# Yukun-Huang/DreamWaltz-G

Measured on AMD Instinct MI355X. Metric: SDS steps/sec @512^2, 100k Gaussians, SD1.5+ControlNet; raster Mpix/s vs HBM roofline, higher is better.
Workload: dtype f32x

## Files before the change

### dreamwaltz-g_amd/csrc/gemm.hip

```cpp
#include "dwg_common.h"
#include "dwg_prof_internal.h"
#include "../../include/dwg_gemm.h"
#include <cstdlib>
#include <type_traits>

#if defined(DWG_GEMM_X_TU)
#include "dwg_xfmt.h"
typedef _Float16 HT;
#define DWG_DTYPE_HALF DWG_DTYPE_F32X
#define DWG_MFMA16(a, b, c) __builtin_amdgcn_mfma_f32_32x32x16_f16(a, b, c, 0, 0, 0)
#define DWG_HALF_NAME "f32x"
#elif defined(DWG_GEMM_F16_TU)
typedef _Float16 HT;
#define DWG_DTYPE_HALF DWG_DTYPE_F16
#define DWG_MFMA16(a, b, c) __builtin_amdgcn_mfma_f32_32x32x16_f16(a, b, c, 0, 0, 0)
#define DWG_HALF_NAME "f16"
#else
typedef __bf16 HT;
#define DWG_DTYPE_HALF DWG_DTYPE_BF16
#define DWG_MFMA16(a, b, c) __builtin_amdgcn_mfma_f32_32x32x16_bf16(a, b, c, 0, 0, 0)
#define DWG_HALF_NAME "bf16"
#endif

namespace {

typedef __attribute__((ext_vector_type(8))) HT bf16x8;
typedef __attribute__((ext_vector_type(16))) float f32x16;

struct ConvP {
    int enabled, Cin, Hin, Win, Hout, Wout, KH, KW, stride, pad_t, pad_l, dil;
    int up;
    int cin1;
    const void* A2;
};

struct GemmP {
    const void* A; const void* B; void* C; const void* bias; const void* residual;
    int M, N, K;
    long long sam, sak, sbn, sbk, ldc, ldr;
    int nb2;
    long long bA1, bA2, bB1, bB2, bC1, bC2, bR1, bR2;
    int act; float alpha;
    int out_bf16, res_bf16, bias_per_row, splitk, accumulate;
    float* ws;
    int bias_row_div;
    long long bias_ld;
    ConvP conv;
};

__device__ __forceinline__ float bf2f(HT x) { return (float)x; }
__device__ __forceinline__ HT f2bf(float x) { return (HT)x; }

struct bf16x4_t { HT v[4]; };
#ifdef DWG_GEMM_X_TU
__device__ __forceinline__ float ld_half1(const void* base, long long i) { return dwg_x_get1(base, i); }
__device__ __forceinline__ void st_half1(void* base, long long i, float v) { dwg_x_put1(base, i, v); }
__device__ __forceinline__ void ld_half4(const void* base, long long i, float (&v)[4]) { dwg_x_get4(base, i, v); }
__device__ __forceinline__ void st_half4(void* base, long long i, const float (&v)[4]) { dwg_x_put4(base, i, v); }
#else
__device__ __forceinline__ float ld_half1(const void* base, long long i) { return bf2f(reinterpret_cast<const HT*>(base)[i]); }
__device__ __forceinline__ void st_half1(void* base, long long i, float v) { reinterpret_cast<HT*>(base)[i] = f2bf(v); }
__device__ __forceinline__ void ld_half4(const void* base, long long i, float (&v)[4]) {
    const bf16x4_t r = *reinterpret_cast<const bf16x4_t*>(reinterpret_cast<const HT*>(base) + i);
#pragma unroll
    for (int e = 0; e < 4; e++) v[e] = bf2f(r.v[e]);
}
__device__ __forceinline__ void st_half4(void* base, long long i, const float (&v)[4]) {
    bf16x4_t o;
#pragma unroll
    for (int e = 0; e < 4; e++) o.v[e] = f2bf(v[e]);
    *reinterpret_cast<bf16x4_t*>(reinterpret_cast<HT*>(base) + i) = o;
}
#endif

template <bool LIGHT = false>
__device__ __forceinline__ float apply_act(float v, int act) {
    if constexpr (LIGHT) return act == 3 ? v / (1.f + __expf(-v)) : v;
    switch (act) {
        case 1: return v > 0.f ? v : 0.f;
        case 2: return v > 0.f ? v : 0.01f * v;
        case 3: return v / (1.f + __expf(-v));
        case 4: return 0.5f * v * (1.f + erff(v * 0.70710678118654752f));
        case 5: return 1.f / (1.f + __expf(-v));
        default: return v;
    }
// ... 1058 lines not shown
                if (TAP0 || tap <= NBS - 2) {
                    constexpr int N = (NBS - 2) * NJW + PPW;
                    __builtin_amdgcn_s_waitcnt((N & 15) | ((N >> 4) << 14) | (7 << 4) | (0 << 8));
                } else {
                    constexpr int N = (NBS - 2) * NJW;
                    __builtin_amdgcn_s_waitcnt((N & 15) | ((N >> 4) << 14) | (7 << 4) | (0 << 8));
                }
                __builtin_amdgcn_s_barrier();
                const int ntap = tap == 8 ? 0 : tap + 1;
                const int nty = ntap >= 6 ? 2 : (ntap >= 3 ? 1 : 0);
                load_frags(tap == 8 ? pan : pa, nty * WP + (ntap - 3 * nty), sB + bnext * BBYTES, 0, F[0]);
            }
            __builtin_amdgcn_sched_barrier(0);
            if (ks == 0) {
                const int ft = tap + NBS - 1, fcc = cc + (ft >= 9 ? 1 : 0), ftap = ft >= 9 ? ft - 9 : ft;
                issue_w(fcc, ftap, fcc < ncc, sB + bfill * BBYTES);
                if (TAP0) issue_patch(cc + 1, cc + 1 < ncc, const_cast<unsigned char*>(pan));
            }
            mma(F[ks & 1]);
            if (ks == 0) {
                constexpr int NL = NJW + (TAP0 ? PPW : 0);
#pragma unroll
                for (int m = 0; m < MPS; m++) {
                    __builtin_amdgcn_sched_group_barrier(0x008, 1, 0);
                    __builtin_amdgcn_sched_group_barrier(0x006, (NL * 8 + MPS - 1) / MPS, 0);
                    __builtin_amdgcn_sched_group_barrier(0x020, (NL + MPS - 1) / MPS, 0);
                }
            }
            __builtin_amdgcn_sched_barrier(0);
        }
        __builtin_amdgcn_s_waitcnt(0xC07F);
        bst = bnext;
    };
    for (int cc = cc0; cc < ncc; cc++) {
        const unsigned char* pa = sP + (cc & 1) * PBYTES;
        const unsigned char* pan = sP + ((cc + 1) & 1) * PBYTES;
        step(BoolC<true>{}, 0, cc, pa, pan);
#pragma unroll 1
        for (int tap = 1; tap < 9; tap++) step(BoolC<false>{}, tap, cc, pa, pan);
    }
    wait_vmcnt<0>();
    __builtin_amdgcn_s_barrier();
#ifdef DWG_GEMM_X_TU
#pragma unroll
    for (int i = 0; i < TM; i++)
#pragma unroll
        for (int j = 0; j < TN; j++)
#pragma unroll
            for (int r = 0; r < 16; r++) acc[i][j][r] = fmaf(acx[i][j][r], DWG_X_LO_INV, acc[i][j][r]);
#endif
    constexpr int NPASS = EpiLds<BN, BM>::passes((size_t)2 * PBYTES + NBS * BBYTES);
    static_assert((size_t)2 * PBYTES + NBS * BBYTES >= EpiLds<BN, BM>::bytes(NPASS), "epilogue staging fits in the patch / weight buffers");
    tile_epilogue_lds<BN, NPASS, TM, TN, !SPLIT, BM, NT>(p, acc, reinterpret_cast<float*>(smem_raw), n0, wm, wn, lane, tid, ks_id, 0, 0, [&](int rr) {
        const int y = y0 + rr / PW, x = x0 + rr % PW;
        return (y < cv.Hout && x < cv.Wout) ? (img * cv.Hout + y) * cv.Wout + x : -1;
    });
}

template <int BN, int NW, int NBS>
static void launch_conv3x3_patch2(const GemmP& p, hipStream_t stream, const char* name) {
    typedef Patch2Geom<BN, NW> G;
    const size_t lds = (size_t)2 * G::PBYTES + (size_t)NBS * G::BBYTES;
    const ConvP& cv = p.conv;
    const int nimg = p.M / (cv.Hout * cv.Wout);
    const int gm = nimg * ((cv.Hout + G::PH - 1) / G::PH) * ((cv.Wout + G::PW - 1) / G::PW);
    dim3 grid(gm * ((p.N + BN - 1) / BN) * (p.splitk > 1 ? p.splitk : 1));
    static bool attr_set = false;
    if (!attr_set) {
        hipFuncSetAttribute(reinterpret_cast<const void*>(&k_conv3x3_patch2<BN, false, NW, NBS>), hipFuncAttributeMaxDynamicSharedMemorySize, (int)lds);
        hipFuncSetAttribute(reinterpret_cast<const void*>(&k_conv3x3_patch2<BN, true, NW, NBS>), hipFuncAttributeMaxDynamicSharedMemorySize, (int)lds);
        attr_set = true;
    }
    static_assert((NW == 8 && BN == 128 && NBS == 4) || (NW == 4 && BN == 64 && NBS == 4) || (NW == 4 && BN == 128 && NBS == 2), "symbol table below");
    const char* sym = NW == 8 ? (p.splitk > 1 && p.ws ? "k_conv3x3_patch2<128, true, 8, 4>" : "k_conv3x3_patch2<128, false, 8, 4>")
                              : (BN == 64 ? (p.splitk > 1 && p.ws ? "k_conv3x3_patch2<64, true, 4, 4>" : "k_conv3x3_patch2<64, false, 4, 4>")
                                          : (p.splitk > 1 && p.ws ? "k_conv3x3_patch2<128, true, 4, 2>" : "k_conv3x3_patch2<128, false, 4, 2>"));
    if (p.splitk > 1 && p.ws)
        DWG_LAUNCH_W(name, sym, gemm_flops(p, 1), (k_conv3x3_patch2<BN, true, NW, NBS>), grid, dim3(NW * 64), lds, stream, p);
    else
        DWG_LAUNCH_W(name, sym, gemm_flops(p, 1), (k_conv3x3_patch2<BN, false, NW, NBS>), grid, dim3(NW * 64), lds, stream, p);
    launch_splitk_epilogue(p, stream);
}

template <typename T, int BN, int AMODE, int BMODE>
static void launch(const GemmP& p, int batch, hipStream_t stream, const char* name) {
    constexpr int LDT = TT<T>::BK + TT<T>::PAD;
    size_t lds = (size_t)2 * (128 + BN) * LDT * sizeof(T);
    dim3 grid((p.M + 127) / 128, ((p.N + BN - 1) / BN) * (p.splitk > 1 ? p.splitk : 1), batch);
    static bool attr_set = false;
    if (!attr_set) {
        hipFuncSetAttribute(reinterpret_cast<const void*>(&k_gemm<T, BN, AMODE, BMODE>), hipFuncAttributeMaxDynamicSharedMemorySize,
                            (int)lds);
        attr_set = true;
    }
    DWG_LAUNCH_W(name, (sizeof(T) == 2 ? "k_gemm<" DWG_HALF_NAME ">" : "k_gemm<f32>"), gemm_flops(p, batch), (k_gemm<T, BN, AMODE, BMODE>), grid,
                 dim3(256), lds, stream, p);
    launch_splitk_epilogue(p, stream);
}

template <typename T, int BN, int AMODE>
static void dispatch_b(const GemmP& p, int bmode, int batch, hipStream_t s, const char* name) {
    if (bmode == MODE_KVEC) launch<T, BN, AMODE, MODE_KVEC>(p, batch, s, name);
    else if (bmode == MODE_RVEC) launch<T, BN, AMODE, MODE_RVEC>(p, batch, s, name);
    else launch<T, BN, AMODE, MODE_SCALAR>(p, batch, s, name);
}
template <typename T, int BN>
static void dispatch_a(const GemmP& p, int amode, int bmode, int batch, hipStream_t s, const char* name) {
    if (amode == MODE_KVEC) dispatch_b<T, BN, MODE_KVEC>(p, bmode, batch, s, name);
    else if (amode == MODE_RVEC) dispatch_b<T, BN, MODE_RVEC>(p, bmode, batch, s, name);
    else if (amode == MODE_CONV) dispatch_b<T, BN, MODE_CONV>(p, bmode, batch, s, name);
    else dispatch_b<T, BN, MODE_SCALAR>(p, bmode, batch, s, name);
}

static int batch_of(const dwg_gemm_desc* d) { return d->batch1 * d->batch2; }

static int tile_bn(const dwg_gemm_desc* d) {
    if (d->N <= 64) return 64;
    const long long blocks128 = (long long)((d->M + 127) / 128) * ((d->N + 127) / 128) * batch_of(d);
    return blocks128 < 256 ? 64 : 128;
}

constexpr int kCUs = 256, kMinWgs = 200;
static bool fills_cus(long long wgs) {
    const long long rounds = (wgs + kCUs - 1) / kCUs;
    return wgs >= kMinWgs && wgs * 100 >= rounds * kCUs * 80;
}

constexpr int kSplitkTarget = 256;
constexpr int kSplitkNoSplit = 384;
constexpr int kSplitkMinSteps = 12;
static int auto_splitk(int M, int N, int K, int bn, int bk) {
    long long blocks = (long long)((M + 127) / 128) * ((N + bn - 1) / bn);
    if (blocks >= kSplitkNoSplit || K < 2 * kSplitkMinSteps * bk) return 1;
    if (2.0 * M * N * K < 4.0e8) return 1;
    long long sk = kSplitkTarget / blocks;
    long long kmax = K / (kSplitkMinSteps * bk);
    if (sk > kmax) sk = kmax;
    if (sk > 16) sk = 16;
    return sk >= 2 ? (int)sk : 1;
}

constexpr int kBigMinK = 1280, kBigMaxTiles = 2048;
constexpr int kBigMinSteps = 8, kBigSkMax = 24;
static int big_tile(int M, int N, int K, int* splitk_out) {
    *splitk_out = 1;
    if (K < kBigMinK) return 0;
    int bm = 0;
    if (M >= 192) { if (N >= 128 && (N % 128 == 0 || N >= 640)) bm = 256; }
    else if (N >= 256) bm = 128;
    if (!bm) return 0;
    const int bn = bm == 256 ? 128 : 256;
    const long long tiles = (long long)((M + bm - 1) / bm) * ((N + bn - 1) / bn);
    if (tiles > kBigMaxTiles) return 0;
    long long sk = 1;
    if (tiles < kCUs) {
        sk = kCUs / tiles;
        const long long kmax = K / (kBigMinSteps * 64);
        if (sk > kmax) sk = kmax;
        if (sk > kBigSkMax) sk = kBigSkMax;
        if (sk < 1) sk = 1;
    }
    if (!fills_cus(tiles * sk)) return 0;
    *splitk_out = (int)sk;
    return bm;
}

template <typename T>
static int pick_mode(const void* base, long long srow, long long sk, int nrows, int K, const long long* boffs, int nboffs) {
    constexpr int VEC = TT<T>::VEC;
    bool aligned = ((uintptr_t)base % 16) == 0;
    for (int i = 0; i < nboffs; i++) aligned = aligned && (boffs[i] % VEC == 0);
    if (sk == 1 && aligned && K % VEC == 0 && srow % VEC == 0) return MODE_KVEC;
    if (srow == 1 && aligned && nrows % VEC == 0 && sk % VEC == 0) return MODE_RVEC;
    return MODE_SCALAR;
}

static int splitk_of(const dwg_gemm_desc* d) {
    if (d->splitk > 1) return d->splitk;
    if (d->splitk != 0 || d->act == DWG_ACT_GEGLU_PAIR) return 1;
    return auto_splitk(d->M, d->N, d->K, tile_bn(d), d->dtype == DWG_DTYPE_HALF ? TT<HT>::BK : TT<float>::BK);
}
static bool slabs_possible(const dwg_gemm_desc* d) { return batch_of(d) == 1 && (long long)d->M * d->N < (1LL << 33); }
static long long fit_workspace(const dwg_gemm_desc* d, long long sk) {
    while (sk > 1 && (size_t)sk * d->M * d->N * sizeof(float) > d->workspace_bytes) sk--;
    return sk;
}

enum Family { FAM_GENERIC, FAM_GLDS, FAM_GLDS8, FAM_PATCH2 };
struct Plan {
    Family fam;
    int bm, bn, nw;
    int amode, bmode;
    int akind;
    int splitk;
    bool slabs;
};

constexpr int kPatchMinM = 8192;
constexpr int kPatch8MinSteps = 100;

static int make_plan(const dwg_gemm_desc* d, const GemmP& p, Plan& pl) {
    const bool half = d->dtype == DWG_DTYPE_HALF;
#if defined(DWG_GEMM_F16_TU) || defined(DWG_GEMM_X_TU)
    if (!half) return DWG_E_ARG;
#endif
    pl = Plan{FAM_GENERIC, 128, tile_bn(d), 4, MODE_KVEC, MODE_KVEC, 0, d->splitk > 1 ? d->splitk : 1, false};
    if (d->workspace && slabs_possible(d)) {
        pl.splitk = (int)fit_workspace(d, splitk_of(d));
        pl.slabs = pl.splitk > 1;
    }
    const long long ao[2] = {p.bA1, p.bA2}, bo[2] = {p.bB1, p.bB2};
    if (p.conv.enabled) {
        const int vec = half ? TT<HT>::VEC : TT<float>::VEC;
        if (d->conv_cin % vec != 0 || ((uintptr_t)d->A % 16) != 0) return DWG_E_ARG;
        if (d->A2 && (d->conv_cin1 % vec != 0 || d->conv_cin1 <= 0 || d->conv_cin1 >= d->conv_cin || ((uintptr_t)d->A2 % 16) != 0))
            return DWG_E_ARG;
        if (d->K != d->conv_kh * d->conv_kw * d->conv_cin) return DWG_E_ARG;
        pl.amode = MODE_CONV;
    } else {
        pl.amode = half ? pick_mode<HT>(p.A, p.sam, p.sak, p.M, p.K, ao, 2) : pick_mode<float>(p.A, p.sam, p.sak, p.M, p.K, ao, 2);
    }
    pl.bmode = half ? pick_mode<HT>(p.B, p.sbn, p.sbk, p.N, p.K, bo, 2) : pick_mode<float>(p.B, p.sbn, p.sbk, p.N, p.K, bo, 2);
    if (!half) return DWG_OK;
    if (pl.bmode != MODE_KVEC || (pl.amode != MODE_KVEC && pl.amode != MODE_CONV)) {
#ifdef DWG_GEMM_X_TU
        return DWG_E_ARG;
#else
        return DWG_OK;
#endif
    }
    const ConvP& cv = p.conv;
    const char* minm = getenv("DWG_CONV_PATCH_MINM");
    const int patch_min_m = minm ? atoi(minm) : kPatchMinM;
    const bool patch_geom = pl.amode == MODE_CONV && batch_of(d) == 1 && d->conv_kh == 3 && d->conv_kw == 3 && d->conv_stride == 1 &&
                            cv.dil == 1 && cv.up == 1 && d->conv_pad_t == 1 && d->conv_pad_l == 1 && !d->A2 && d->conv_cin % 64 == 0 &&
                            d->conv_hout == d->conv_hin && d->conv_wout == d->conv_win && d->conv_wout >= 16 && d->conv_hout >= 8;
    const int ncc = d->conv_cin / 64;
    if (patch_geom && d->splitk <= 1 && d->conv_hout % 16 == 0 && d->conv_wout % 16 == 0 && (d->N % 128 == 0 || d->N >= 512)) {
        const long long tiles8 = (long long)(d->M / 256) * ((d->N + 127) / 128);
        long long sk = 1;
        if (tiles8 < kMinWgs && d->workspace && d->splitk == 0 && slabs_possible(d)) {
            sk = kCUs / tiles8;
            if (sk > ncc / 2) sk = ncc / 2;
            sk = fit_workspace(d, sk);
            if (sk < 1) sk = 1;
            const long long per = (ncc + sk - 1) / sk;
            sk = (ncc + per - 1) / per;
        }
        const long long steps = (ncc + sk - 1) / sk * 9;
        const bool worth = sk > 1 || steps >= kPatch8MinSteps || d->M < patch_min_m;
        if (worth && fills_cus(tiles8 * sk) && (d->act == 0 || d->act == 3 || sk > 1)) {
            pl = Plan{FAM_PATCH2, 256, 128, 8, MODE_CONV, pl.bmode, 0, (int)sk, sk > 1};
            return DWG_OK;
        }
    }
    if (patch_geom && d->M >= patch_min_m && (d->act == 0 || d->act == 3 || pl.splitk > 1)) {
        if (pl.splitk > 1) {
            const int gm = (d->M / (d->conv_hout * d->conv_wout)) * ((d->conv_hout + 7) / 8) * ((d->conv_wout + 15) / 16);
            const int blocks = gm * ((d->N + pl.bn - 1) / pl.bn);
            int sk = blocks >= 256 ? 1 : (384 + blocks - 1) / blocks;
            if (sk > ncc / 2) sk = ncc / 2;
            if (sk > pl.splitk) sk = pl.splitk;
            if (sk < 2) sk = 1;
            pl.splitk = sk;
            pl.slabs = pl.slabs && sk > 1;
        }
        pl.fam = FAM_PATCH2;
        return DWG_OK;
    }
    const bool fast_geom = pl.amode == MODE_CONV && d->conv_cin % 64 == 0 && cv.dil == 1 && cv.up == 1 && d->conv_kh * d->conv_kw <= 32;
    const bool cat_fast = d->A2 && d->conv_cin1 % 64 == 0 && (d->conv_cin - d->conv_cin1) % 64 == 0;
    pl.akind = pl.amode != MODE_CONV ? 0 : (fast_geom && !d->A2 ? 2 : (fast_geom && cat_fast ? 3 : 1));
    int big_sk = 1;
    const int big_bm = d->splitk <= 1 ? big_tile(d->M, d->N, d->K, &big_sk) : 0;
    if (big_bm) {
        if (d->act == DWG_ACT_GEGLU_PAIR || !d->workspace || !slabs_possible(d) || d->splitk == 1) big_sk = 1;
        big_sk = (int)fit_workspace(d, big_sk);
        const int bbn = big_bm == 256 ? 128 : 256;
        const long long tiles = (long long)((d->M + big_bm - 1) / big_bm) * ((d->N + bbn - 1) / bbn) * batch_of(d);
        if (fills_cus(tiles * big_sk)) {
            pl = Plan{FAM_GLDS8, big_bm, bbn, 8, pl.amode, pl.bmode, pl.akind, big_sk, big_sk > 1};
            return DWG_OK;
        }
    }
    pl.fam = FAM_GLDS;
    return DWG_OK;
}

template <typename T>
static void launch_generic(const GemmP& p, const Plan& pl, int batch, hipStream_t s, const char* name) {
    if (pl.bn == 64) dispatch_a<T, 64>(p, pl.amode, pl.bmode, batch, s, name);
    else dispatch_a<T, 128>(p, pl.amode, pl.bmode, batch, s, name);
}
template <typename F>
static void with_akind(int akind, F f) {
    if (akind == 3) f(std::integral_constant<int, 3>{});
    else if (akind == 2) f(std::integral_constant<int, 2>{});
    else if (akind == 1) f(std::integral_constant<int, 1>{});
    else f(std::integral_constant<int, 0>{});
}

}

#ifdef DWG_GEMM_X_TU
static bool x_physical(const dwg_gemm_desc* d, dwg_gemm_desc* o) {
    if (!d) return false;
    *o = *d;
    if (d->dtype != DWG_DTYPE_F32X) return false;
    if (d->K % 8 || d->a_k_stride != 1 || d->b_k_stride != 1) return false;
    if ((d->a_row_stride | d->b_row_stride | d->a_batch1_stride | d->a_batch2_stride | d->b_batch1_stride | d->b_batch2_stride) % 8) return false;
    if (d->out_dtype == DWG_DTYPE_F32X && ((d->ldc | d->c_batch1_stride | d->c_batch2_stride) % 8 || ((uintptr_t)d->C % 16))) return false;
    if (d->residual && d->residual_dtype == DWG_DTYPE_F32X &&
        (((d->ldr ? d->ldr : d->ldc) | d->r_batch1_stride | d->r_batch2_stride) % 8 || ((uintptr_t)d->residual % 16))) return false;
    if (d->act == DWG_ACT_GEGLU_PAIR && d->out_dtype == DWG_DTYPE_F32X && d->N % 16) return false;
    if (d->conv_enabled && (d->conv_cin % 8 || (d->A2 && d->conv_cin1 % 8))) return false;
    o->K = 2 * d->K;
    o->a_row_stride = 2 * d->a_row_stride; o->b_row_stride = 2 * d->b_row_stride;
    o->a_batch1_stride = 2 * d->a_batch1_stride; o->a_batch2_stride = 2 * d->a_batch2_stride;
    o->b_batch1_stride = 2 * d->b_batch1_stride; o->b_batch2_stride = 2 * d->b_batch2_stride;
    o->conv_cin = 2 * d->conv_cin; o->conv_cin1 = 2 * d->conv_cin1;
    return true;
}
#endif

extern "C" {

#if defined(DWG_GEMM_X_TU)
#define DWG_GEMM_FN dwg_gemm_x
#define DWG_GEMM_WS_FN dwg_gemm_workspace_bytes_x
#elif defined(DWG_GEMM_F16_TU)
#define DWG_GEMM_FN dwg_gemm_f16
#define DWG_GEMM_WS_FN dwg_gemm_workspace_bytes_f16
#else
#define DWG_GEMM_FN dwg_gemm
#define DWG_GEMM_WS_FN dwg_gemm_workspace_bytes
size_t dwg_gemm_workspace_bytes_f16(const dwg_gemm_desc* d);
int dwg_gemm_f16(const dwg_gemm_desc* d, dwg_stream_t stream);
size_t dwg_gemm_workspace_bytes_x(const dwg_gemm_desc* d);
int dwg_gemm_x(const dwg_gemm_desc* d, dwg_stream_t stream);
#endif

size_t DWG_GEMM_WS_FN(const dwg_gemm_desc* d) {
#if !defined(DWG_GEMM_F16_TU) && !defined(DWG_GEMM_X_TU)
    if (d && d->dtype == DWG_DTYPE_F16) return dwg_gemm_workspace_bytes_f16(d);
    if (d && d->dtype == DWG_DTYPE_F32X) return dwg_gemm_workspace_bytes_x(d);
#endif
#ifdef DWG_GEMM_X_TU
    dwg_gemm_desc xd;
    if (!x_physical(d, &xd)) return 0;
    d = &xd;
#endif
    if (!d || d->M <= 0 || d->N <= 0 || !slabs_possible(d)) return 0;
    dwg_gemm_desc pd = *d;
    if (d->plan_m > d->M) pd.M = d->plan_m;
    d = &pd;
    int sk = splitk_of(d);
    if (d->dtype == DWG_DTYPE_HALF && d->splitk == 0 && d->act != DWG_ACT_GEGLU_PAIR) {
        int bsk = 1;
        if (big_tile(d->M, d->N, d->K, &bsk) && bsk > sk) sk = bsk;
    }
    return sk > 1 ? (size_t)sk * d->M * d->N * sizeof(float) : 0;
}

int DWG_GEMM_FN(const dwg_gemm_desc* d, dwg_stream_t stream_) {
#if !defined(DWG_GEMM_F16_TU) && !defined(DWG_GEMM_X_TU)
    if (d && d->dtype == DWG_DTYPE_F16) return dwg_gemm_f16(d, stream_);
    if (d && d->dtype == DWG_DTYPE_F32X) return dwg_gemm_x(d, stream_);
#endif
#ifdef DWG_GEMM_X_TU
    dwg_gemm_desc xd;
    if (!x_physical(d, &xd)) return DWG_E_ARG;
    d = &xd;
#endif
    if (!d || !d->A || !d->B || !d->C) return DWG_E_ARG;
    if (d->M < 0 || d->N < 0 || d->K < 0 || d->batch1 < 1 || d->batch2 < 1 || d->plan_m < 0) return DWG_E_ARG;
    if (d->M == 0 || d->N == 0) return DWG_OK;
    if (d->dtype != DWG_DTYPE_F32 && d->dtype != DWG_DTYPE_HALF) return DWG_E_ARG;
    if (d->splitk > 1 && !d->workspace && (d->out_dtype != DWG_DTYPE_F32 || d->bias || d->residual || d->act)) return DWG_E_ARG;
    if (d->accumulate && d->out_dtype != DWG_DTYPE_F32) return DWG_E_ARG;
    if (d->act == DWG_ACT_GEGLU_PAIR && (d->N % 64 != 0 || d->residual || d->splitk > 1 || d->bias_per_row || d->bias_row_div)) return DWG_E_ARG;
    if ((uintptr_t)d->workspace & 15) return DWG_E_ARG;
    GemmP p;
    p.A = d->A; p.B = d->B; p.C = d->C; p.bias = d->bias; p.residual = d->residual;
    p.M = d->M; p.N = d->N; p.K = d->K;
    p.sam = d->a_row_stride; p.sak = d->a_k_stride; p.sbn = d->b_row_stride; p.sbk = d->b_k_stride;
    p.ldc = d->ldc; p.ldr = d->ldr ? d->ldr : d->ldc;
    p.nb2 = d->batch2;
    p.bA1 = d->a_batch1_stride; p.bA2 = d->a_batch2_stride; p.bB1 = d->b_batch1_stride; p.bB2 = d->b_batch2_stride;
    p.bC1 = d->c_batch1_stride; p.bC2 = d->c_batch2_stride; p.bR1 = d->r_batch1_stride; p.bR2 = d->r_batch2_stride;
    p.act = d->act; p.alpha = d->alpha;
    p.out_bf16 = d->out_dtype == DWG_DTYPE_HALF; p.res_bf16 = d->residual_dtype == DWG_DTYPE_HALF;
    p.bias_per_row = d->bias_per_row; p.accumulate = d->accumulate;
    const bool plain1x1 = d->conv_enabled && d->conv_kh == 1 && d->conv_kw == 1 && d->conv_stride == 1 && d->conv_pad_t == 0 &&
                          d->conv_pad_l == 0 && d->conv_in_dilation <= 1 && d->conv_in_upsample <= 1 && !d->A2 && d->conv_hout == d->conv_hin &&
                          d->conv_wout == d->conv_win && d->K == d->conv_cin && batch_of(d) == 1;
    if (plain1x1) { p.sam = d->conv_cin; p.sak = 1; }
    p.conv.enabled = d->conv_enabled && !plain1x1;
    p.conv.Cin = d->conv_cin; p.conv.Hin = d->conv_hin; p.conv.Win = d->conv_win; p.conv.Hout = d->conv_hout;
    p.conv.Wout = d->conv_wout; p.conv.KH = d->conv_kh; p.conv.KW = d->conv_kw; p.conv.stride = d->conv_stride;
    p.conv.pad_t = d->conv_pad_t; p.conv.pad_l = d->conv_pad_l; p.conv.dil = d->conv_in_dilation > 1 ? d->conv_in_dilation : 1;
    p.conv.up = d->conv_in_upsample > 1 ? d->conv_in_upsample : 1;
    p.conv.A2 = d->A2; p.conv.cin1 = d->A2 ? d->conv_cin1 : d->conv_cin;
    p.bias_row_div = d->bias_row_div; p.bias_ld = d->bias_ld > 0 ? d->bias_ld : d->N;
    Plan pl;
    dwg_gemm_desc pd = *d;
    if (d->plan_m > d->M) pd.M = d->plan_m;
    const int rc = make_plan(&pd, p, pl);
    if (rc != DWG_OK) return rc;
    p.splitk = pl.splitk;
    p.ws = pl.slabs ? reinterpret_cast<float*>(d->workspace) : nullptr;
    const int batch = batch_of(d);
    hipStream_t stream = (hipStream_t)stream_;
    const char* name = d->name ? d->name : (d->conv_enabled ? "conv_igemm" : "gemm");
    switch (pl.fam) {
        case FAM_PATCH2:
            if (pl.nw == 8) launch_conv3x3_patch2<128, 8, 4>(p, stream, name);
            else if (pl.bn == 64) launch_conv3x3_patch2<64, 4, 4>(p, stream, name);
            else launch_conv3x3_patch2<128, 4, 2>(p, stream, name);
            break;
        case FAM_GLDS8:
            with_akind(pl.akind, [&](auto ak) {
                if (pl.bm == 256) launch_glds8<256, 128, decltype(ak)::value>(p, batch, stream, name);
                else launch_glds8<128, 256, decltype(ak)::value>(p, batch, stream, name);
            });
            break;
        case FAM_GLDS:
            with_akind(pl.akind, [&](auto ak) {
                if (pl.bn == 64) launch_glds<64, decltype(ak)::value>(p, batch, stream, name);
                else launch_glds<128, decltype(ak)::value>(p, batch, stream, name);
            });
            break;
        case FAM_GENERIC:
#if defined(DWG_GEMM_X_TU)
            return DWG_E_ARG;
#elif defined(DWG_GEMM_F16_TU)
            launch_generic<HT>(p, pl, batch, stream, name);
#else
            if (d->dtype == DWG_DTYPE_HALF) launch_generic<HT>(p, pl, batch, stream, name);
            else launch_generic<float>(p, pl, batch, stream, name);
#endif
            break;
    }
    DWG_RETURN_IF_LAUNCH_FAILED();
    return DWG_OK;
}

}
```

Measured before the change: 42.12.

## Add specialized thin-channel 3x3 conv kernels for Cin=8 and Cout=8

Adds two dedicated MFMA kernels for 3x3 stride-1 convolutions whose channel count is tiny: one for 8 input channels (the latent-in conv, e.g. ControlNet hint or VAE-like input) and one for 8 output channels (the output conv). The generic implicit-GEMM path wastes most of a K or N tile on such shapes. The Cin=8 kernel keeps weights in registers and packs taps into the K dimension. The Cout=8 kernel stages a halo patch and the weights in LDS and uses 16x16 MFMAs. Both bypass split-K and workspace, and they add new code paths plus a static attribute-set flag that is not thread-safe.

Result: no change. 42.26 (median of 5 runs) (+0.3%).

```diff
diff --git a/dreamwaltz-g_amd/csrc/conv_thin.h b/dreamwaltz-g_amd/csrc/conv_thin.h
--- /dev/null
+++ b/dreamwaltz-g_amd/csrc/conv_thin.h
@@ -0,0 +1,19 @@
+#pragma once
+#include <hip/hip_runtime.h>
+
+struct dwg_conv_thin_p {
+    const void* A;
+    const void* B;
+    void* C;
+    const float* bias;
+    int M;
+    int H, W, Cin, N;
+    long long ldc;
+    int dtype;
+    int out_f32;
+    int act;
+    float alpha;
+};
+
+void dwg_conv3x3_cin8_launch(const dwg_conv_thin_p& p, hipStream_t stream, const char* name);
+void dwg_conv3x3_cout8_launch(const dwg_conv_thin_p& p, hipStream_t stream, const char* name);
diff --git a/dreamwaltz-g_amd/csrc/conv_thin.hip b/dreamwaltz-g_amd/csrc/conv_thin.hip
--- /dev/null
+++ b/dreamwaltz-g_amd/csrc/conv_thin.hip
@@ -0,0 +1,269 @@
+#include "dwg_common.h"
+#include "dwg_prof_internal.h"
+#include "dwg_xfmt.h"
+#include "conv_thin.h"
+#include "../../include/dwg_gemm.h"
+
+namespace {
+
+typedef float f4 __attribute__((ext_vector_type(4)));
+typedef float f16v __attribute__((ext_vector_type(16)));
+
+template <typename T> struct ET {
+    typedef T H;
+    static constexpr int BYTES = 16;
+    static constexpr bool X = false;
+};
+template <> struct ET<dwg_xs> {
+    typedef _Float16 H;
+    static constexpr int BYTES = 32;
+    static constexpr bool X = true;
+};
+template <typename H> struct Frag { typedef H type __attribute__((ext_vector_type(8))); };
+
+__device__ __forceinline__ f16v mfma32(Frag<_Float16>::type a, Frag<_Float16>::type b, f16v c) {
+    return __builtin_amdgcn_mfma_f32_32x32x16_f16(a, b, c, 0, 0, 0);
+}
+__device__ __forceinline__ f16v mfma32(Frag<__bf16>::type a, Frag<__bf16>::type b, f16v c) {
+    return __builtin_amdgcn_mfma_f32_32x32x16_bf16(a, b, c, 0, 0, 0);
+}
+__device__ __forceinline__ f4 mfma16(Frag<_Float16>::type a, Frag<_Float16>::type b, f4 c) {
+    return __builtin_amdgcn_mfma_f32_16x16x32_f16(a, b, c, 0, 0, 0);
+}
+__device__ __forceinline__ f4 mfma16(Frag<__bf16>::type a, Frag<__bf16>::type b, f4 c) {
+    return __builtin_amdgcn_mfma_f32_16x16x32_bf16(a, b, c, 0, 0, 0);
+}
+
+template <typename T> struct Operand {
+    typedef typename Frag<typename ET<T>::H>::type frag;
+    frag hi, lo;
+    __device__ __forceinline__ void zero() {
+#pragma unroll
+        for (int e = 0; e < 8; e++) { hi[e] = 0; lo[e] = 0; }
+    }
+    __device__ __forceinline__ void load(const unsigned char* p) {
+        hi = *reinterpret_cast<const frag*>(p);
+        if constexpr (ET<T>::X) lo = *reinterpret_cast<const frag*>(p + 16);
+    }
+};
+
+template <typename T, int NV>
+__device__ __forceinline__ void store_cols(const dwg_conv_thin_p& p, long long m, int col, const float (&v)[NV]) {
+    static_assert(NV == 4 || NV == 8, "whole 8- or 16-byte pieces");
+    const long long i = m * p.ldc + col;
+    if (p.out_f32) {
+        float* o = reinterpret_cast<float*>(p.C) + i;
+#pragma unroll
+        for (int e = 0; e < NV; e += 4) *reinterpret_cast<f4*>(o + e) = f4{v[e], v[e + 1], v[e + 2], v[e + 3]};
+    } else if constexpr (ET<T>::X && NV == 8) {
+        dwg_x8 g;
+#pragma unroll
+        for (int e = 0; e < 8; e++) g.set(e, v[e]);
+        g.store(reinterpret_cast<dwg_xs*>(p.C) + i);
+    } else if constexpr (ET<T>::X) {
+        dwg_x_put4(p.C, i, v);
+    } else {
+        typedef T vec __attribute__((ext_vector_type(NV)));
+        vec r;
+#pragma unroll
+        for (int e = 0; e < NV; e++) r[e] = (T)v[e];
+        *reinterpret_cast<vec*>(reinterpret_cast<T*>(p.C) + i) = r;
+    }
+}
+
+constexpr int kC8Pix = 32, kC8Cols = 128, kC8LD = kC8Cols + 4;
+
+template <typename T>
+__global__ __launch_bounds__(256, 2) void k_conv3x3_cin8(dwg_conv_thin_p p, int iters) {
+    __shared__ __attribute__((aligned(16))) float stage[kC8Pix * kC8LD];
+    constexpr int GB = ET<T>::BYTES;
+    const int tid = threadIdx.x, lane = tid & 63, r = lane & 31, h = lane >> 5, wv = tid >> 6;
+    const int col0 = blockIdx.y * kC8Cols, cb = col0 + wv * 32;
+    const unsigned char* A = reinterpret_cast<const unsigned char*>(p.A);
+    const unsigned char* B = reinterpret_cast<const unsigned char*>(p.B);
+    Operand<T> w[5];
+#pragma unroll
+    for (int ks = 0; ks < 5; ks++) {
+        const int t = 2 * ks + h;
+        w[ks].zero();
+        if (t < 9 && cb + r < p.N) w[ks].load(B + ((size_t)(cb + r) * 9 + t) * GB);
+    }
+    float bias[16];
+#pragma unroll
+    for (int j = 0; j < 16; j++) {
+        const int c = cb + (j & 3) + 8 * (j >> 2) + 4 * h;
+        bias[j] = p.bias && c < p.N ? p.bias[c] : 0.f;
+    }
+    const int H = p.H, W = p.W, HW = H * W;
+    const int G = min(16, (p.N - col0) >> 3);
+    Operand<T> xs[5];
+    auto fetch = [&](long long t0) {
+        const long long m = t0 + r;
+        const int pix = (int)(m % HW), y = pix / W, x = pix - y * W;
+#pragma unroll
+        for (int ks = 0; ks < 5; ks++) {
+            const int t = 2 * ks + h, dy = t / 3 - 1, dx = t - (dy + 1) * 3 - 1;
+            xs[ks].zero();
+            if (t < 9 && m < p.M && (unsigned)(y + dy) < (unsigned)H && (unsigned)(x + dx) < (unsigned)W)
+                xs[ks].load(A + (size_t)(m + dy * W + dx) * GB);
+        }
+    };
+    fetch((long long)blockIdx.x * iters * kC8Pix);
+    for (int it = 0; it < iters; it++) {
+        const long long m0 = ((long long)blockIdx.x * iters + it) * kC8Pix;
+        if (m0 >= p.M) break;
+        f16v main, cross;
+#pragma unroll
+        for (int j = 0; j < 16; j++) { main[j] = 0.f; cross[j] = 0.f; }
+        if (cb < p.N) {
+#pragma unroll
+            for (int ks = 0; ks < 5; ks++) {
+                main = mfma32(w[ks].hi, xs[ks].hi, main);
+                if constexpr (ET<T>::X) {
+                    cross = mfma32(w[ks].lo, xs[ks].hi, cross);
+                    cross = mfma32(w[ks].hi, xs[ks].lo, cross);
+                }
+            }
+        }
+        if (it + 1 < iters) fetch(m0 + kC8Pix);
+        if (cb < p.N) {
+#pragma unroll
+            for (int i = 0; i < 4; i++) {
+                f4 o;
+#pragma unroll
+                for (int e = 0; e < 4; e++) {
+                    float v = main[4 * i + e];
+                    if constexpr (ET<T>::X) v = __builtin_fmaf(cross[4 * i + e], DWG_X_LO_INV, v);
+                    v = v * p.alpha + bias[4 * i + e];
+                    o[e] = p.act == DWG_ACT_SILU ? v / (1.f + __expf(-v)) : v;
+                }
+                *reinterpret_cast<f4*>(stage + r * kC8LD + wv * 32 + 8 * i + 4 * h) = o;
+            }
+        }
+        __syncthreads();
+        for (int i = tid; i < kC8Pix * G; i += 256) {
+            const int px = i / G, g = i - px * G;
+            if (m0 + px >= p.M) continue;
+            const f4 a = *reinterpret_cast<const f4*>(stage + px * kC8LD + g * 8), b = *reinterpret_cast<const f4*>(stage + px * kC8LD + g * 8 + 4);
+            const float v[8] = {a[0], a[1], a[2], a[3], b[0], b[1], b[2], b[3]};
+            store_cols<T, 8>(p, m0 + px, col0 + g * 8, v);
+        }
+        __syncthreads();
+    }
+}
+
+constexpr int kT8H = 8, kT8W = 16, kT8WP = kT8W + 2, kT8NPIX = (kT8H + 2) * kT8WP;
+template <typename T> constexpr int cout8_pixel_stride() { return 8 * ET<T>::BYTES + 16; }
+template <typename T> constexpr size_t cout8_lds() { return (size_t)kT8NPIX * cout8_pixel_stride<T>() + 9 * 8 * 8 * ET<T>::BYTES; }
+
+template <typename T>
+__global__ __launch_bounds__(256, 2) void k_conv3x3_cout8(dwg_conv_thin_p p) {
+    extern __shared__ __attribute__((aligned(16))) unsigned char patch[];
+    constexpr int GB = ET<T>::BYTES, CPP = 8 * GB / 16, PS = cout8_pixel_stride<T>();
+    unsigned char* wl = patch + kT8NPIX * PS;
+    const int tid = threadIdx.x, lane = tid & 63, c = lane & 15, q = lane >> 4, wv = tid >> 6;
+    const int H = p.H, W = p.W, Cin = p.Cin, img = blockIdx.z, ty0 = blockIdx.y * kT8H, tx0 = blockIdx.x * kT8W;
+    const unsigned char* A = reinterpret_cast<const unsigned char*>(p.A);
+    const unsigned char* B = reinterpret_cast<const unsigned char*>(p.B);
+    f4 main[2], cross[2];
+#pragma unroll
+    for (int rt = 0; rt < 2; rt++)
+#pragma unroll
+        for (int e = 0; e < 4; e++) { main[rt][e] = 0.f; cross[rt][e] = 0.f; }
+    for (int slab = 0; slab < Cin / 64; slab++) {
+        __syncthreads();
+        for (int i = tid; i < kT8NPIX * CPP; i += 256) {
+            const int px = i / CPP, ch = i - px * CPP, py = px / kT8WP, iy = ty0 + py - 1, ix = tx0 + (px - py * kT8WP) - 1;
+            uint4 v = {0u, 0u, 0u, 0u};
+            if ((unsigned)iy < (unsigned)H && (unsigned)ix < (unsigned)W)
+                v = *reinterpret_cast<const uint4*>(A + ((((size_t)img * H + iy) * W + ix) * Cin + slab * 64) * (GB / 8) + ch * 16);
+            *reinterpret_cast<uint4*>(patch + px * PS + ch * 16) = v;
+        }
+        for (int i = tid; i < 8 * 9 * 8 * (GB / 16); i += 256) {
+            const int ch = i % (GB / 16), g = (i / (GB / 16)) & 7, t = (i / (GB / 16) >> 3) % 9, n = i / (GB / 16) / 72;
+            *reinterpret_cast<uint4*>(wl + ((t * 8 + g) * 8 + n) * GB + ch * 16) =
+                *reinterpret_cast<const uint4*>(B + (((size_t)n * 9 + t) * Cin + slab * 64 + g * 8) * (GB / 8) + ch * 16);
+        }
+        __syncthreads();
+#pragma unroll
+        for (int t = 0; t < 9; t++) {
+            const int dy = t / 3, dx = t - dy * 3;
+#pragma unroll
+            for (int k2 = 0; k2 < 2; k2++) {
+                const int g = 4 * k2 + q;
+                Operand<T> wf;
+                wf.zero();
+                if (c < 8) wf.load(wl + ((t * 8 + g) * 8 + c) * GB);
+#pragma unroll
+                for (int rt = 0; rt < 2; rt++) {
+                    Operand<T> xf;
+                    xf.load(patch + ((2 * wv + rt + dy) * kT8WP + c + dx) * PS + g * GB);
+                    main[rt] = mfma16(wf.hi, xf.hi, main[rt]);
+                    if constexpr (ET<T>::X) {
+                        cross[rt] = mfma16(wf.lo, xf.hi, cross[rt]);
+                        cross[rt] = mfma16(wf.hi, xf.lo, cross[rt]);
+                    }
+                }
+            }
+        }
+    }
+    if (q >= 2) return;
+#pragma unroll
+    for (int rt = 0; rt < 2; rt++) {
+        const int y = ty0 + 2 * wv + rt, x = tx0 + c;
+        const long long m = ((long long)img * H + y) * W + x;
+        if (y >= H || x >= W || m >= p.M) continue;
+        float v[4];
+#pragma unroll
+        for (int e = 0; e < 4; e++) {
+            v[e] = main[rt][e];
+            if constexpr (ET<T>::X) v[e] = __builtin_fmaf(cross[rt][e], DWG_X_LO_INV, v[e]);
+            v[e] *= p.alpha;
+        }
+        store_cols<T, 4>(p, m, 4 * q, v);
+    }
+}
+
+template <typename T> struct Sym;
+template <> struct Sym<__bf16> { static constexpr const char* cin8 = "k_conv3x3_cin8<__bf16>"; static constexpr const char* cout8 = "k_conv3x3_cout8<__bf16>"; };
+template <> struct Sym<_Float16> { static constexpr const char* cin8 = "k_conv3x3_cin8<_Float16>"; static constexpr const char* cout8 = "k_conv3x3_cout8<_Float16>"; };
+template <> struct Sym<dwg_xs> { static constexpr const char* cin8 = "k_conv3x3_cin8<dwg_xs>"; static constexpr const char* cout8 = "k_conv3x3_cout8<dwg_xs>"; };
+
+static double thin_flops(const dwg_conv_thin_p& p) { return 2.0 * p.M * p.N * 9.0 * p.Cin; }
+
+template <typename T>
+static void launch_cin8(const dwg_conv_thin_p& p, hipStream_t stream, const char* name) {
+    const int ncol = dwg_cdiv(p.N, kC8Cols);
+    const long long tiles = ((long long)p.M + kC8Pix - 1) / kC8Pix;
+    long long iters = (tiles * ncol + 767) / 768;
+    iters = iters < 1 ? 1 : (iters > 16 ? 16 : iters);
+    dim3 grid((unsigned)((tiles + iters - 1) / iters), ncol, 1);
+    DWG_LAUNCH_W(name, Sym<T>::cin8, thin_flops(p), (k_conv3x3_cin8<T>), grid, dim3(256), 0, stream, p, (int)iters);
+}
+
+template <typename T>
+static void launch_cout8(const dwg_conv_thin_p& p, hipStream_t stream, const char* name) {
+    constexpr size_t lds = cout8_lds<T>();
+    static bool attr_set = false;
+    if (!attr_set) {
+        hipFuncSetAttribute(reinterpret_cast<const void*>(&k_conv3x3_cout8<T>), hipFuncAttributeMaxDynamicSharedMemorySize, (int)lds);
+        attr_set = true;
+    }
+    const long long hw = (long long)p.H * p.W;
+    dim3 grid(dwg_cdiv(p.W, kT8W), dwg_cdiv(p.H, kT8H), (unsigned)((p.M + hw - 1) / hw));
+    DWG_LAUNCH_W(name, Sym<T>::cout8, thin_flops(p), (k_conv3x3_cout8<T>), grid, dim3(256), lds, stream, p);
+}
+
+}
+
+void dwg_conv3x3_cin8_launch(const dwg_conv_thin_p& p, hipStream_t stream, const char* name) {
+    if (p.dtype == DWG_DTYPE_F32X) launch_cin8<dwg_xs>(p, stream, name);
+    else if (p.dtype == DWG_DTYPE_F16) launch_cin8<_Float16>(p, stream, name);
+    else launch_cin8<__bf16>(p, stream, name);
+}
+
+void dwg_conv3x3_cout8_launch(const dwg_conv_thin_p& p, hipStream_t stream, const char* name) {
+    if (p.dtype == DWG_DTYPE_F32X) launch_cout8<dwg_xs>(p, stream, name);
+    else if (p.dtype == DWG_DTYPE_F16) launch_cout8<_Float16>(p, stream, name);
+    else launch_cout8<__bf16>(p, stream, name);
+}
diff --git a/dreamwaltz-g_amd/csrc/gemm.hip b/dreamwaltz-g_amd/csrc/gemm.hip
--- a/dreamwaltz-g_amd/csrc/gemm.hip
+++ b/dreamwaltz-g_amd/csrc/gemm.hip
@@ -1,6 +1,7 @@
 #include "dwg_common.h"
 #include "dwg_prof_internal.h"
 #include "../../include/dwg_gemm.h"
+#include "conv_thin.h"
 #include <cstdlib>
 #include <type_traits>
 
@@ -1329,7 +1330,7 @@
     return sk;
 }
 
-enum Family { FAM_GENERIC, FAM_GLDS, FAM_GLDS8, FAM_PATCH2 };
+enum Family { FAM_GENERIC, FAM_GLDS, FAM_GLDS8, FAM_PATCH2, FAM_THIN_CIN8, FAM_THIN_COUT8 };
 struct Plan {
     Family fam;
     int bm, bn, nw;
@@ -1341,6 +1342,25 @@
 
 constexpr int kPatchMinM = 8192;
 constexpr int kPatch8MinSteps = 100;
+
+#ifdef DWG_GEMM_X_TU
+constexpr int kHalvesPerElement = 2;
+#else
+constexpr int kHalvesPerElement = 1;
+#endif
+static Family thin_family(const dwg_gemm_desc* d) {
+    if (d->dtype != DWG_DTYPE_HALF || !d->conv_enabled || batch_of(d) != 1) return FAM_GENERIC;
+    if (d->conv_kh != 3 || d->conv_kw != 3 || d->conv_stride != 1 || d->conv_pad_t != 1 || d->conv_pad_l != 1 || d->conv_in_dilation > 1 ||
+        d->conv_in_upsample > 1 || d->A2 || d->conv_hout != d->conv_hin || d->conv_wout != d->conv_win || d->conv_hin < 1 || d->conv_win < 1)
+        return FAM_GENERIC;
+    if (d->K != 9 * d->conv_cin || d->a_k_stride != 1 || d->b_k_stride != 1 || d->b_row_stride != d->K) return FAM_GENERIC;
+    if (d->residual || d->bias_per_row || d->bias_row_div || d->accumulate || d->splitk > 1) return FAM_GENERIC;
+    if (d->act != DWG_ACT_NONE && d->act != DWG_ACT_SILU) return FAM_GENERIC;
+    if ((((uintptr_t)d->A | (uintptr_t)d->B | (uintptr_t)d->C) & 15) || d->N % 8 || d->ldc % 8) return FAM_GENERIC;
+    if (d->conv_cin == 8 * kHalvesPerElement) return FAM_THIN_CIN8;
+    if (d->N == 8 && d->conv_cin % (64 * kHalvesPerElement) == 0 && !d->bias && d->act == DWG_ACT_NONE) return FAM_THIN_COUT8;
+    return FAM_GENERIC;
+}
 
 static int make_plan(const dwg_gemm_desc* d, const GemmP& p, Plan& pl) {
     const bool half = d->dtype == DWG_DTYPE_HALF;
@@ -1371,6 +1391,11 @@
 #else
         return DWG_OK;
 #endif
+    }
+    const Family thin = thin_family(d);
+    if (thin != FAM_GENERIC) {
+        pl = Plan{thin, 0, 0, 4, MODE_CONV, MODE_KVEC, 0, 1, false};
+        return DWG_OK;
     }
     const ConvP& cv = p.conv;
     const char* minm = getenv("DWG_CONV_PATCH_MINM");
@@ -1493,7 +1518,7 @@
     if (!x_physical(d, &xd)) return 0;
     d = &xd;
 #endif
-    if (!d || d->M <= 0 || d->N <= 0 || !slabs_possible(d)) return 0;
+    if (!d || d->M <= 0 || d->N <= 0 || !slabs_possible(d) || thin_family(d) != FAM_GENERIC) return 0;
     dwg_gemm_desc pd = *d;
     if (d->plan_m > d->M) pd.M = d->plan_m;
     d = &pd;
@@ -1561,6 +1586,16 @@
             else if (pl.bn == 64) launch_conv3x3_patch2<64, 4, 4>(p, stream, name);
             else launch_conv3x3_patch2<128, 4, 2>(p, stream, name);
             break;
+        case FAM_THIN_CIN8:
+        case FAM_THIN_COUT8: {
+            dwg_conv_thin_p t;
+            t.A = d->A; t.B = d->B; t.C = d->C; t.bias = d->bias;
+            t.M = d->M; t.H = d->conv_hin; t.W = d->conv_win; t.Cin = d->conv_cin / kHalvesPerElement; t.N = d->N;
+            t.ldc = d->ldc; t.dtype = DWG_DTYPE_HALF; t.out_f32 = !p.out_bf16; t.act = d->act; t.alpha = d->alpha;
+            if (pl.fam == FAM_THIN_CIN8) dwg_conv3x3_cin8_launch(t, stream, name);
+            else dwg_conv3x3_cout8_launch(t, stream, name);
+            break;
+        }
         case FAM_GLDS8:
             with_akind(pl.akind, [&](auto ak) {
                 if (pl.bm == 256) launch_glds8<256, 128, decltype(ak)::value>(p, batch, stream, name);
```

## Add specialized thin-channel 3x3 conv kernels for f32x input and output layers

Applied to the files above, without the earlier changes.

Adds two dedicated 3x3 stride-1 conv kernels for the split-precision (f32x) path. The first targets 16-input-channel convs and the second 8-output-channel convs, the shapes of the first and last layers of the UNet/ControlNet. Each stages a haloed spatial patch in LDS and runs small MFMA tiles with hi/lo compensation terms. The aim is to avoid the generic implicit-GEMM path, which wastes tile work and bandwidth on these skinny K or N shapes. The routing applies only above an M threshold and for restricted epilogues (no residual, accumulate, or per-row bias).

Result: no change. 39.87 before, 40.13 after (median of 6 runs) (+0.6%).

```diff
diff --git a/dreamwaltz-g_amd/csrc/conv_thin_x.h b/dreamwaltz-g_amd/csrc/conv_thin_x.h
--- /dev/null
+++ b/dreamwaltz-g_amd/csrc/conv_thin_x.h
@@ -0,0 +1,224 @@
+#pragma once
+
+typedef __attribute__((ext_vector_type(4))) float f32x4;
+
+__device__ __forceinline__ bf16x8 thin_zero8() { return bf16x8{(HT)0.f, (HT)0.f, (HT)0.f, (HT)0.f, (HT)0.f, (HT)0.f, (HT)0.f, (HT)0.f}; }
+
+struct ThinIn {
+    static constexpr int PH = 8, PW = 32, WP = PW + 2, NPIX = (PH + 2) * WP, BN = 128;
+    static constexpr int SROW = BN * 4 + 16;
+};
+
+__global__ __launch_bounds__(256) void k_conv3x3_thin_in(GemmP p) {
+    typedef ThinIn G;
+    __shared__ __attribute__((aligned(16))) unsigned char sHi[G::NPIX * 16];
+    __shared__ __attribute__((aligned(16))) unsigned char sLo[G::NPIX * 16];
+    __shared__ __attribute__((aligned(16))) unsigned char sOut[2][32 * G::SROW];
+    const ConvP& cv = p.conv;
+    const int tid = threadIdx.x, lane = tid & 63, wave = tid >> 6;
+    const int H = cv.Hout, W = cv.Wout;
+    const int tiles_x = (W + G::PW - 1) / G::PW, tiles_y = (H + G::PH - 1) / G::PH, ntn = (p.N + G::BN - 1) / G::BN;
+    const int mt = blockIdx.x / ntn, n0 = (blockIdx.x % ntn) * G::BN;
+    const int img = mt / (tiles_y * tiles_x), trem = mt % (tiles_y * tiles_x);
+    const int y0 = (trem / tiles_x) * G::PH, x0 = (trem % tiles_x) * G::PW;
+    const HT* X = reinterpret_cast<const HT*>(p.A) + (long long)img * H * W * 16;
+    const HT* Wt = reinterpret_cast<const HT*>(p.B);
+
+    for (int c = tid; c < G::NPIX * 2; c += 256) {
+        const int pix = c >> 1, half = c & 1;
+        const int py = pix / G::WP, px = pix - py * G::WP;
+        const int iy = y0 - 1 + py, ix = x0 - 1 + px;
+        uint4 v = make_uint4(0u, 0u, 0u, 0u);
+        if (iy >= 0 && iy < H && ix >= 0 && ix < W) v = *reinterpret_cast<const uint4*>(X + ((long long)iy * W + ix) * 16 + half * 8);
+        *reinterpret_cast<uint4*>((half ? sLo : sHi) + pix * 16) = v;
+    }
+
+    const int col0 = n0 + wave * 32;
+    const bool active = col0 < p.N;
+    const int h = lane >> 5, pl = lane & 31;
+    bf16x8 bh[5], bl[5];
+    {
+        const int i = lane & 31;
+        const int c = col0 + 16 * ((i >> 2) & 1) + 4 * (i >> 3) + (i & 3);
+#pragma unroll
+        for (int ks = 0; ks < 5; ks++) {
+            const int t = 2 * ks + h;
+            bh[ks] = thin_zero8(); bl[ks] = thin_zero8();
+            if (c < p.N && t < 9) {
+                const HT* w = Wt + (long long)c * p.sbn + t * 16;
+                bh[ks] = *reinterpret_cast<const bf16x8*>(w);
+                bl[ks] = *reinterpret_cast<const bf16x8*>(w + 8);
+            }
+        }
+    }
+    float bias[16];
+#pragma unroll
+    for (int r = 0; r < 16; r++) {
+        const int c = col0 + 16 * h + r;
+        bias[r] = (p.bias && c < p.N) ? reinterpret_cast<const float*>(p.bias)[c] : 0.f;
+    }
+    int aoff[5];
+#pragma unroll
+    for (int ks = 0; ks < 5; ks++) {
+        const int t = 2 * ks + h, tt = t < 9 ? t : 0;
+        aoff[ks] = ((tt / 3) * G::WP + pl + tt % 3) * 16;
+    }
+    __syncthreads();
+
+#pragma unroll 1
+    for (int by = 0; by < G::PH; by++) {
+        unsigned char* so = sOut[by & 1];
+        if (active) {
+            f32x16 acc, acx;
+#pragma unroll
+            for (int r = 0; r < 16; r++) { acc[r] = 0.f; acx[r] = 0.f; }
+#pragma unroll
+            for (int ks = 0; ks < 5; ks++) {
+                bf16x8 ah = *reinterpret_cast<const bf16x8*>(sHi + by * G::WP * 16 + aoff[ks]);
+                bf16x8 al = *reinterpret_cast<const bf16x8*>(sLo + by * G::WP * 16 + aoff[ks]);
+                if (ks == 4 && h) { ah = thin_zero8(); al = thin_zero8(); }
+                acc = DWG_MFMA16(bh[ks], ah, acc);
+                acx = DWG_MFMA16(bl[ks], ah, acx);
+                acx = DWG_MFMA16(bh[ks], al, acx);
+            }
+            dwg_h8 oh[2], ol[2];
+#pragma unroll
+            for (int r = 0; r < 16; r++) {
+                float v = fmaf(fmaf(acx[r], DWG_X_LO_INV, acc[r]), p.alpha, bias[r]);
+                v = apply_act<true>(v, p.act);
+                _Float16 a, b;
+                dwg_x_split(v, a, b);
+                oh[r >> 3][r & 7] = a; ol[r >> 3][r & 7] = b;
+            }
+            unsigned char* dst = so + pl * G::SROW + (wave * 32 + 16 * h) * 4;
+            *reinterpret_cast<dwg_h8*>(dst) = oh[0];
+            *reinterpret_cast<dwg_h8*>(dst + 16) = ol[0];
+            *reinterpret_cast<dwg_h8*>(dst + 32) = oh[1];
+            *reinterpret_cast<dwg_h8*>(dst + 48) = ol[1];
+        }
+        __syncthreads();
+        const int y = y0 + by;
+        if (y < H) {
+#pragma unroll
+            for (int q = 0; q < 4; q++) {
+                const int id = q * 256 + tid, pr = id >> 5, ch = id & 31;
+                const int x = x0 + pr;
+                if (x < W && n0 + (ch >> 1) * 8 < p.N) {
+                    const long long row = ((long long)img * H + y) * W + x;
+                    unsigned char* out = reinterpret_cast<unsigned char*>(p.C) + (row * p.ldc + n0) * 4 + ch * 16;
+                    *reinterpret_cast<uint4*>(out) = *reinterpret_cast<const uint4*>(so + pr * G::SROW + ch * 16);
+                }
+            }
+        }
+    }
+}
+
+static void launch_conv3x3_thin_in(const GemmP& p, hipStream_t stream, const char* name) {
+    typedef ThinIn G;
+    const ConvP& cv = p.conv;
+    const int nimg = p.M / (cv.Hout * cv.Wout);
+    dim3 grid(nimg * ((cv.Hout + G::PH - 1) / G::PH) * ((cv.Wout + G::PW - 1) / G::PW) * ((p.N + G::BN - 1) / G::BN));
+    DWG_LAUNCH_W(name, "k_conv3x3_thin_in", gemm_flops(p, 1), k_conv3x3_thin_in, grid, dim3(256), 0, stream, p);
+}
+
+struct ThinOut {
+    static constexpr int PH = 16, PW = 16, WP = PW + 2, NPIX = (PH + 2) * WP;
+    static constexpr int SLAB = 64;
+    static constexpr int SPIX = SLAB * 2 + 16;
+    static constexpr int NCHUNK = NPIX * 8, CPT = (NCHUNK + 255) / 256;
+};
+
+__global__ __launch_bounds__(256) void k_conv3x3_thin_out(GemmP p) {
+    typedef ThinOut G;
+    __shared__ __attribute__((aligned(16))) unsigned char sP[G::NPIX * G::SPIX];
+    const ConvP& cv = p.conv;
+    const int tid = threadIdx.x, lane = tid & 63, wave = tid >> 6;
+    const int H = cv.Hout, W = cv.Wout, Cin = cv.Cin;
+    const int tiles_x = (W + G::PW - 1) / G::PW, tiles_y = (H + G::PH - 1) / G::PH;
+    const int img = blockIdx.x / (tiles_y * tiles_x), trem = blockIdx.x % (tiles_y * tiles_x);
+    const int y0 = (trem / tiles_x) * G::PH, x0 = (trem % tiles_x) * G::PW;
+    const HT* X = reinterpret_cast<const HT*>(p.A) + (long long)img * H * W * Cin;
+    const HT* Wt = reinterpret_cast<const HT*>(p.B);
+    const int ngroups = Cin / 16, nslabs = (Cin + G::SLAB - 1) / G::SLAB;
+    const int lp = lane & 15, kq = lane >> 4;
+    const HT* wrow = Wt + (long long)(lane & 7) * p.sbn + kq * 16 + ((lane >> 3) & 1) * 8;
+
+    long long psrc[G::CPT];
+    int pdst[G::CPT];
+#pragma unroll
+    for (int j = 0; j < G::CPT; j++) {
+        const int c = tid + j * 256, pix = c >> 3, ch = c & 7;
+        const int py = pix / G::WP, px = pix - py * G::WP;
+        const int iy = y0 - 1 + py, ix = x0 - 1 + px;
+        const bool ok = c < G::NCHUNK && iy >= 0 && iy < H && ix >= 0 && ix < W;
+        psrc[j] = ok ? ((long long)iy * W + ix) * Cin + ch * 8 : -1;
+        pdst[j] = c < G::NCHUNK ? pix * G::SPIX + ch * 16 : -1;
+    }
+    f32x4 acc1[4], acc2[4];
+#pragma unroll
+    for (int g = 0; g < 4; g++)
+#pragma unroll
+        for (int r = 0; r < 4; r++) { acc1[g][r] = 0.f; acc2[g][r] = 0.f; }
+
+#pragma unroll 1
+    for (int s = 0; s < nslabs; s++) {
+        const bool gok = s * 4 + kq < ngroups;
+        bf16x8 wf[9];
+#pragma unroll
+        for (int t = 0; t < 9; t++) wf[t] = gok ? *reinterpret_cast<const bf16x8*>(wrow + (long long)t * Cin + s * G::SLAB) : thin_zero8();
+        uint4 pv[G::CPT];
+#pragma unroll
+        for (int j = 0; j < G::CPT; j++) {
+            const int ch = (tid + j * 256) & 7;
+            pv[j] = (psrc[j] >= 0 && s * 4 + (ch >> 1) < ngroups) ? *reinterpret_cast<const uint4*>(X + psrc[j] + s * G::SLAB)
+                                                                 : make_uint4(0u, 0u, 0u, 0u);
+        }
+        __syncthreads();
+#pragma unroll
+        for (int j = 0; j < G::CPT; j++)
+            if (pdst[j] >= 0) *reinterpret_cast<uint4*>(sP + pdst[j]) = pv[j];
+        __syncthreads();
+#pragma unroll
+        for (int g = 0; g < 4; g++) {
+            const unsigned char* base = sP + ((wave * 4 + g) * G::WP + lp) * G::SPIX + kq * 32;
+#pragma unroll
+            for (int t = 0; t < 9; t++) {
+                const unsigned char* a = base + ((t / 3) * G::WP + t % 3) * G::SPIX;
+                const bf16x8 ah = *reinterpret_cast<const bf16x8*>(a);
+                const bf16x8 al = *reinterpret_cast<const bf16x8*>(a + 16);
+                acc1[g] = __builtin_amdgcn_mfma_f32_16x16x32_f16(wf[t], ah, acc1[g], 0, 0, 0);
+                acc2[g] = __builtin_amdgcn_mfma_f32_16x16x32_f16(wf[t], al, acc2[g], 0, 0, 0);
+            }
+        }
+    }
+
+    const int c4 = (lane >> 4) * 4;
+    const float* bias = reinterpret_cast<const float*>(p.bias);
+#pragma unroll
+    for (int g = 0; g < 4; g++) {
+        float v[4];
+#pragma unroll
+        for (int r = 0; r < 4; r++) {
+            const float hl = __shfl(acc1[g][r], (lane + 32) & 63);
+            v[r] = fmaf(hl + acc2[g][r], DWG_X_LO_INV, acc1[g][r]) * p.alpha;
+        }
+        const int y = y0 + wave * 4 + g, x = x0 + lp;
+        if (lane < 32 && y < H && x < W) {
+            if (bias) {
+#pragma unroll
+                for (int r = 0; r < 4; r++) v[r] += bias[c4 + r];
+            }
+            const long long ci = (((long long)img * H + y) * W + x) * p.ldc + c4;
+            if (p.out_bf16) st_half4(p.C, ci, v);
+            else *reinterpret_cast<float4*>(reinterpret_cast<float*>(p.C) + ci) = make_float4(v[0], v[1], v[2], v[3]);
+        }
+    }
+}
+
+static void launch_conv3x3_thin_out(const GemmP& p, hipStream_t stream, const char* name) {
+    typedef ThinOut G;
+    const ConvP& cv = p.conv;
+    const int nimg = p.M / (cv.Hout * cv.Wout);
+    dim3 grid(nimg * ((cv.Hout + G::PH - 1) / G::PH) * ((cv.Wout + G::PW - 1) / G::PW));
+    DWG_LAUNCH_W(name, "k_conv3x3_thin_out", gemm_flops(p, 1), k_conv3x3_thin_out, grid, dim3(256), 0, stream, p);
+}
diff --git a/dreamwaltz-g_amd/csrc/gemm.hip b/dreamwaltz-g_amd/csrc/gemm.hip
--- a/dreamwaltz-g_amd/csrc/gemm.hip
+++ b/dreamwaltz-g_amd/csrc/gemm.hip
@@ -1225,6 +1225,10 @@
     launch_splitk_epilogue(p, stream);
 }
 
+#ifdef DWG_GEMM_X_TU
+#include "conv_thin_x.h"
+#endif
+
 template <typename T, int BN, int AMODE, int BMODE>
 static void launch(const GemmP& p, int batch, hipStream_t stream, const char* name) {
     constexpr int LDT = TT<T>::BK + TT<T>::PAD;
@@ -1329,7 +1333,7 @@
     return sk;
 }
 
-enum Family { FAM_GENERIC, FAM_GLDS, FAM_GLDS8, FAM_PATCH2 };
+enum Family { FAM_GENERIC, FAM_GLDS, FAM_GLDS8, FAM_PATCH2, FAM_THIN_IN, FAM_THIN_OUT };
 struct Plan {
     Family fam;
     int bm, bn, nw;
@@ -1340,6 +1344,7 @@
 };
 
 constexpr int kPatchMinM = 8192;
+constexpr long long kThinMinM = 65536;
 constexpr int kPatch8MinSteps = 100;
 
 static int make_plan(const dwg_gemm_desc* d, const GemmP& p, Plan& pl) {
@@ -1373,6 +1378,26 @@
 #endif
     }
     const ConvP& cv = p.conv;
+#ifdef DWG_GEMM_X_TU
+    {
+        const char* tmin = getenv("DWG_CONV_THIN_MINM");
+        const long long thin_min_m = tmin ? atoll(tmin) : kThinMinM;
+        const bool thin_geom = pl.amode == MODE_CONV && batch_of(d) == 1 && d->conv_kh == 3 && d->conv_kw == 3 && d->conv_stride == 1 &&
+                               cv.dil == 1 && cv.up == 1 && d->conv_pad_t == 1 && d->conv_pad_l == 1 && !d->A2 &&
+                               d->conv_hout == d->conv_hin && d->conv_wout == d->conv_win && d->splitk <= 1 && !d->residual && !d->accumulate &&
+                               !d->bias_per_row && d->bias_row_div == 0 && d->M >= thin_min_m &&
+                               p.M % (d->conv_hout * d->conv_wout) == 0;
+        const bool out_x = d->out_dtype == DWG_DTYPE_HALF;
+        if (thin_geom && d->conv_cin == 16 && d->N % 8 == 0 && out_x && (d->act == 0 || d->act == 3)) {
+            pl.fam = FAM_THIN_IN; pl.splitk = 1; pl.slabs = false;
+            return DWG_OK;
+        }
+        if (thin_geom && d->N == 8 && d->conv_cin % 16 == 0 && d->act == 0 && (out_x || (d->ldc % 4 == 0 && (uintptr_t)d->C % 16 == 0))) {
+            pl.fam = FAM_THIN_OUT; pl.splitk = 1; pl.slabs = false;
+            return DWG_OK;
+        }
+    }
+#endif
     const char* minm = getenv("DWG_CONV_PATCH_MINM");
     const int patch_min_m = minm ? atoi(minm) : kPatchMinM;
     const bool patch_geom = pl.amode == MODE_CONV && batch_of(d) == 1 && d->conv_kh == 3 && d->conv_kw == 3 && d->conv_stride == 1 &&
@@ -1561,6 +1586,13 @@
             else if (pl.bn == 64) launch_conv3x3_patch2<64, 4, 4>(p, stream, name);
             else launch_conv3x3_patch2<128, 4, 2>(p, stream, name);
             break;
+#ifdef DWG_GEMM_X_TU
+        case FAM_THIN_IN: launch_conv3x3_thin_in(p, stream, name); break;
+        case FAM_THIN_OUT: launch_conv3x3_thin_out(p, stream, name); break;
+#else
+        case FAM_THIN_IN:
+        case FAM_THIN_OUT: return DWG_E_ARG;
+#endif
         case FAM_GLDS8:
             with_akind(pl.akind, [&](auto ak) {
                 if (pl.bm == 256) launch_glds8<256, 128, decltype(ak)::value>(p, batch, stream, name);
```
